# CristianSimion5/vk-raytracing-engine

Hardware: AMD Instinct MI355X
Metric: Mrays/s (higher is better)
Workload: dtype f32

## Files before the change

vk-raytracing-engine_amd/csrc/shade.h:

```cpp
#pragma once
#include "device_math.h"
#include "device_scene.h"
#include "texel.h"
#include "traverse.h"

struct Payload
{
  f3 hitValue;
  uint32_t seed;
  uint32_t depth;
  f3 rayOrigin, rayDirection, weight;
  bool isSpecular;
  float lightDist;
  f3 shadowRayDir;
};

struct ShadeStats
{
  unsigned hits, diffuse, taps;
  const float* lut;
};

VKRT_DEV const float* ldsTexelLut(const DevScene& sc, float* lds512)
{
  for(unsigned i = threadIdx.x; i < 512u; i += blockDim.x)
    lds512[i] = sc.srgbLut[i];
  __syncthreads();
  return lds512;
}

VKRT_DEV ShadeStats shadeStatsInit(const DevScene& sc, float* lds512)
{
  ShadeStats st;
  st.hits = 0; st.diffuse = 0; st.taps = 0;
  st.lut = ldsTexelLut(sc, lds512);
  return st;
}

VKRT_DEV f4 sampleTexLevel(const DevScene& sc, const DevTexture& tx, const uint32_t* levelOffsets, uint32_t level, float u, float v, const float* lut)
{
  const uint32_t ws = tx.width >> level, hs = tx.height >> level;
  const uint32_t w = ws ? ws : 1u, h = hs ? hs : 1u;
  TexTap tp;
  texFootprint(level == 0u ? tx.offset : levelOffsets[level], w, h, (tx.srgb & 1u) != 0u, true, true, u, v, tp);
  return texBlend(lut, tp, sc.texels[tp.i00], sc.texels[tp.i10], sc.texels[tp.i01], sc.texels[tp.i11]);
}

VKRT_DEV float lodLog2(float x)
{
  const uint32_t b = (uint32_t)__float_as_int(x);
  int e = (int)((b >> 23) & 255u) - 127;
  float m = __int_as_float((int)((b & 0x007fffffu) | 0x3f800000u));
  if(m > 1.41421356f)
  {
    m = m * 0.5f;
    e += 1;
  }
  const float s = (m - 1.0f) / (m + 1.0f), s2 = s * s;
  const float series = 1.0f + s2 * (0.333333333f + s2 * (0.2f + s2 * (0.142857143f + s2 * 0.111111111f)));
  return (float)e + (2.0f * s * series) * 1.44269504f;
}

struct TexGrad
{
  float dudx, dvdx, dudy, dvdy;
  bool on;
};

VKRT_DEV f4 sampleTex(const DevScene& sc, int texIndex, float u, float v, const TexGrad& g, ShadeStats& st)
{
  st.taps++;
  f4 r;
  if(sc.textureCount == 0u || texIndex < 0 || texIndex >= (int)sc.textureCount)
  {
    r.x = r.y = r.z = r.w = 1.0f;
    return r;
  }
  DevTexture tx = sc.textures[texIndex];
  const uint32_t levels = tx.srgb >> 8;
  if(!g.on || levels <= 1u)
    return sampleTexLevel(sc, tx, nullptr, 0u, u, v, st.lut);
  const uint32_t* levelOffsets = sc.texMips + (size_t)texIndex * VKRT_MAX_MIPS;
  const float fw = (float)tx.width, fh = (float)tx.height;
  const float mxu = g.dudx * fw, mxv = g.dvdx * fh, myu = g.dudy * fw, myv = g.dvdy * fh;
  const float rx2 = mxu * mxu + mxv * mxv, ry2 = myu * myu + myv * myv;
  const bool majorX = rx2 >= ry2;
  const float rmax = sqrtf(majorX ? rx2 : ry2), rmin = sqrtf(majorX ? ry2 : rx2);
  float eta = 1.0f;
  if(rmin > 0.0f)
    eta = glsl_min(rmax / rmin, 4.0f);
  else if(rmax > 0.0f)
    eta = 4.0f;
  if(!(eta >= 1.0f))
    eta = 1.0f;
  const int N = (int)ceilf(eta);
  const float scale = rmax / eta;
  float lambda = 0.0f;
  if(scale > 1.0f && scale < 3.0e38f)
    lambda = lodLog2(scale);
  else if(!(scale <= 1.0f))
    lambda = (float)(levels - 1u);
  lambda = glsl_clamp(lambda, 0.0f, (float)(levels - 1u));
  const float fl = floorf(lambda), delta = lambda - fl;
  const uint32_t hi = (uint32_t)fl, lo = hi + 1u < levels ? hi + 1u : levels - 1u;
  const float du = majorX ? g.dudx : g.dudy, dv = majorX ? g.dvdx : g.dvdy;
  r.x = r.y = r.z = r.w = 0.0f;
  for(int i = 1; i <= N; i++)
  {
    const float o = (float)i / (float)(N + 1) - 0.5f;
    float tu = u + o * du, tv = v + o * dv;
    if(!(fabsf(tu) < 1.0e9f) || !(fabsf(tv) < 1.0e9f))
    {
      tu = u;
      tv = v;
    }
    const f4 a = sampleTexLevel(sc, tx, levelOffsets, hi, tu, tv, st.lut), b = sampleTexLevel(sc, tx, levelOffsets, lo, tu, tv, st.lut);
    r.x = r.x + (a.x * (1.0f - delta) + b.x * delta);
    r.y = r.y + (a.y * (1.0f - delta) + b.y * delta);
    r.z = r.z + (a.z * (1.0f - delta) + b.z * delta);
    r.w = r.w + (a.w * (1.0f - delta) + b.w * delta);
  }
  const float inv = 1.0f / (float)N;
  r.x = r.x * inv; r.y = r.y * inv; r.z = r.z * inv; r.w = r.w * inv;
  return r;
}

VKRT_DEV f3 pbrGetBaseColor(const DevScene& sc, const GltfPBRMaterial& mat, float tu, float tv, const TexGrad& g, ShadeStats& st)
{
  f3 color = mk3(mat.pbrBaseColorFactor[0], mat.pbrBaseColorFactor[1], mat.pbrBaseColorFactor[2]);
  if(mat.pbrBaseColorTexture > -1)
  {
    const f4 t = sampleTex(sc, mat.pbrBaseColorTexture, tu, tv, g, st);
    color = color * mk3(t.x, t.y, t.z);
  }
  return color;
}
VKRT_DEV void pbrGetMetallicRoughness(const DevScene& sc, const GltfPBRMaterial& mat, float tu, float tv, const TexGrad& g,
                                      float& metallic, float& roughness, ShadeStats& st)
{
  metallic = mat.metallicFactor;
  roughness = mat.roughnessFactor;
  if(mat.metallicRoughnessTexture > -1)
  {
    const f4 t = sampleTex(sc, mat.metallicRoughnessTexture, tu, tv, g, st);
    roughness *= t.y;
    metallic *= t.z;
  }
}
VKRT_DEV float getNDF_GGXTR(f3 N, f3 H, float alpha)
{
  float a2 = alpha * alpha;
  float NH = dot3(N, H);
  if(NH <= 0.0f)
    return 0.0f;
  float NH2 = NH * NH;
  float d = NH2 * (a2 - 1.0f) + 1.0f;
  return a2 * VKRT_INV_PI / (d * d + 1e-4f);
}
VKRT_DEV float getG_SchlickGGX(float NV, float k) { return NV / (NV * (1.0f - k) + k); }
VKRT_DEV float getG_Smith(f3 N, f3 V, f3 L, float k)
{
  float NV = fabsf(dot3(N, V));
  float NL = fabsf(dot3(N, L));
  return getG_SchlickGGX(NV, k) * getG_SchlickGGX(NL, k);
}
VKRT_DEV f3 getF_Schlick(f3 H, f3 V, f3 F0)
{
  return F0 + (mk3(1.0f) - F0) * vk_pow5(1.0f - fabsf(dot3(H, V)));
}
VKRT_DEV f3 getSpecularBRDF_Cook_Torrance(f3 N, f3 H, f3 V, f3 L, f3 F0, float roughness)
{
  float alpha = roughness * roughness;
  float k = (roughness + 1.0f) * (roughness + 1.0f) / 8.0f;
  float D = getNDF_GGXTR(N, H, alpha);
  float G = getG_Smith(N, V, L, k);
  f3 F = getF_Schlick(H, V, F0);
  float down = 4.0f * fabsf(dot3(V, N)) * fabsf(dot3(L, N)) + 1e-4f;
  return D * F * G / down;
}
VKRT_DEV f3 getSpecularBRDF_over_pdf_Cook_Torrance(f3 N, f3 H, f3 V, f3 L, f3 F0, float roughness, float ratio)
{
  float k = (roughness + 1.0f) * (roughness + 1.0f) / 8.0f;
  float pdf = (1.0f - ratio) * dot3(N, H) / (4.0f * dot3(L, H) + 1e-4f);
  float G = getG_Smith(N, V, L, k);
  f3 F = getF_Schlick(H, V, F0);
  float down = 4.0f * fabsf(dot3(V, N)) * fabsf(dot3(L, N)) + 1e-4f;
  return (F * G / down) / pdf;
}
VKRT_DEV f3 computePBR_BRDF(f3 N, f3 V, f3 L, f3 H, f3 baseColor, float metalness, float roughness)
{
  f3 F0 = mk3(0.04f);
  F0 = glsl_mix(F0, baseColor, metalness);
  f3 F = getF_Schlick(H, V, F0);
  f3 f_cook_torrance = getSpecularBRDF_Cook_Torrance(N, H, V, L, F0, roughness);
  f3 kD = mk3(1.0f) - F;
  kD = kD * (1.0f - metalness);
  f3 f_lambert = baseColor * VKRT_INV_PI;
  f3 diffuse = kD * f_lambert;
  return diffuse + f_cook_torrance;
}
VKRT_DEV f3 directLight(const GltfLight& light, f3 P, f3 N, f3 V, f3 baseColor, float metalness, float roughness, unsigned retap,
                        f3& Li, float& cosTheta, ShadeStats& st)
{
  Li = mk3(0.0f);
  cosTheta = 0.0f;
  if(light.type == 0)
  {
    f3 Ldir = mk3(light.position[0], light.position[1], light.position[2]) - P;
    float d = length3(Ldir);
    f3 L = Ldir / d;
    f3 H = normalize3(L + V);
    float attenuation = d * d;
    Li = mk3(light.color[0], light.color[1], light.color[2]) * light.intensity / attenuation;
    cosTheta = glsl_max(dot3(L, N), 0.0f);
    if(cosTheta > 0.0f)
    {
      st.taps += retap;
      return computePBR_BRDF(N, V, L, H, baseColor, metalness, roughness);
    }
  }
  return mk3(0.0f);
}

VKRT_DEV f3 xformPoint(const DevInstance& in, f3 p)
{
  f3 r;
  r.x = ((in.o2w[0] * p.x + in.o2w[1] * p.y) + in.o2w[2] * p.z) + in.o2w[3];
  r.y = ((in.o2w[4] * p.x + in.o2w[5] * p.y) + in.o2w[6] * p.z) + in.o2w[7];
  r.z = ((in.o2w[8] * p.x + in.o2w[9] * p.y) + in.o2w[10] * p.z) + in.o2w[11];
  return r;
}
VKRT_DEV f3 xformNormal(const DevInstance& in, f3 n)
{
  f3 r;
  r.x = (n.x * in.w2o[0] + n.y * in.w2o[3]) + n.z * in.w2o[6];
  r.y = (n.x * in.w2o[1] + n.y * in.w2o[4]) + n.z * in.w2o[7];
  r.z = (n.x * in.w2o[2] + n.y * in.w2o[5]) + n.z * in.w2o[8];
  return r;
}

struct HitMid
{
  f3 worldPos, N, tangent, binormal, V, baseColor, emittance;
  float metalU, roughU;
  unsigned retap;
};

VKRT_DEV void closestHitFront(const DevScene& sc, const RayHit& hit, const uint32_t instId, const uint4 ts, f3 worldRayDir, const Payload& prd,
                              ShadeStats& st, HitMid& mid)
{
  st.hits++;
  const uint32_t i0 = ts.x, i1 = ts.y, i2 = ts.z, matIndex = ts.w;
  const f3 b = mk3(1.0f - hit.u - hit.v, hit.u, hit.v);

  const BufView vPN = bufView(sc.vertexPN), vMat = bufView(sc.shadeMaterials), vInst = bufView(sc.instances);
  const float4 a0 = bufLoad4(vPN, VKRT_VERTEX_BYTES * i0), b0 = bufLoad4(vPN, VKRT_VERTEX_BYTES * i0 + 16u), tq0 = bufLoad4(vPN, VKRT_VERTEX_BYTES * i0 + 32u);
  const float4 a1 = bufLoad4(vPN, VKRT_VERTEX_BYTES * i1), b1 = bufLoad4(vPN, VKRT_VERTEX_BYTES * i1 + 16u), tq1 = bufLoad4(vPN, VKRT_VERTEX_BYTES * i1 + 32u);
  const float4 a2 = bufLoad4(vPN, VKRT_VERTEX_BYTES * i2), b2 = bufLoad4(vPN, VKRT_VERTEX_BYTES * i2 + 16u), tq2 = bufLoad4(vPN, VKRT_VERTEX_BYTES * i2 + 32u);
  const uint32_t mo = 64u * matIndex;
  const float4 m0 = bufLoad4(vMat, mo), m1 = bufLoad4(vMat, mo + 16u), ref01 = bufLoad4(vMat, mo + 32u), ref23 = bufLoad4(vMat, mo + 48u);
  const uint32_t dimB = __float_as_uint(ref01.x), baseB = __float_as_uint(ref01.y), dimM = __float_as_uint(ref01.z), baseM = __float_as_uint(ref01.w);
  const uint32_t dimN = __float_as_uint(ref23.x), baseN = __float_as_uint(ref23.y), dimE = __float_as_uint(ref23.z), baseE = __float_as_uint(ref23.w);
  DevInstance in;
  {
    const uint32_t io = 96u * instId;
    const float4 q0 = bufLoad4(vInst, io), q1 = bufLoad4(vInst, io + 16u), q2 = bufLoad4(vInst, io + 32u), q3 = bufLoad4(vInst, io + 48u), q4 = bufLoad4(vInst, io + 64u),
                 q5 = bufLoad4(vInst, io + 80u);
    in.o2w[0] = q0.x; in.o2w[1] = q0.y; in.o2w[2] = q0.z; in.o2w[3] = q0.w; in.o2w[4] = q1.x; in.o2w[5] = q1.y; in.o2w[6] = q1.z; in.o2w[7] = q1.w;
    in.o2w[8] = q2.x; in.o2w[9] = q2.y; in.o2w[10] = q2.z; in.o2w[11] = q2.w;
    in.w2o[0] = q3.x; in.w2o[1] = q3.y; in.w2o[2] = q3.z; in.w2o[3] = q3.w; in.w2o[4] = q4.x; in.w2o[5] = q4.y; in.w2o[6] = q4.z; in.w2o[7] = q4.w;
    in.w2o[8] = q5.x; in.primMesh = __float_as_int(q5.y); in.vis = 0u; in.pad = 0;
  }
  GltfPBRMaterial mat;
  mat.pbrBaseColorFactor[0] = m0.x; mat.pbrBaseColorFactor[1] = m0.y; mat.pbrBaseColorFactor[2] = m0.z; mat.pbrBaseColorFactor[3] = 1.0f;
  mat.metallicFactor = m0.w; mat.roughnessFactor = m1.x;
  mat.emissiveFactor[0] = m1.y; mat.emissiveFactor[1] = m1.z; mat.emissiveFactor[2] = m1.w;
  mat.pbrBaseColorTexture = (dimB & 0x8000u) ? 0 : -1; mat.metallicRoughnessTexture = (dimM & 0x8000u) ? 0 : -1;
  mat.normalTexture = (dimN & 0x8000u) ? 0 : -1; mat.emissiveTexture = (dimE & 0x8000u) ? 0 : -1;
  const float tu = (b0.z * b.x + b1.z * b.y) + b2.z * b.z;
  const float tv = (b0.w * b.x + b1.w * b.y) + b2.w * b.z;

  const bool emits = prd.depth == 0 || prd.isSpecular;
  const bool wantE = emits && mat.emissiveTexture > -1, wantN = mat.normalTexture > -1;
  const bool wantB = mat.pbrBaseColorTexture > -1, wantM = mat.metallicRoughnessTexture > -1;
  st.taps += (wantE ? 1u : 0u) + (wantN ? 1u : 0u) + (wantB ? 1u : 0u) + (wantM ? 1u : 0u);
  TexTap tE, tN, tB, tM;
#define VKRT_FOOTPRINT(dim, base, want, tap)                                                                                           \
  texFootprint(sc.texQuads ? 0u : ((base) & 0x7fffffffu), ((dim) & 0x7fffu) + 1u, (((dim) >> 16) & 0x7fffu) + 1u, ((base) >> 31) != 0u, \
               ((dim) >> 31) != 0u, want, tu, tv, tap)
  VKRT_FOOTPRINT(dimE, baseE, wantE, tE);
  VKRT_FOOTPRINT(dimN, baseN, wantN, tN);
  VKRT_FOOTPRINT(dimB, baseB, wantB, tB);
  VKRT_FOOTPRINT(dimM, baseM, wantM, tM);
#undef VKRT_FOOTPRINT
  uint32_t e00, e10, e01, e11, n00, n10, n01, n11, c00, c10, c01, c11, r00, r10, r01, r11;
  if(sc.texQuads)
  {
    const BufView quads = bufView(sc.texQuads);
#define VKRT_QUAD(dim, base, tap, want, a, b, c, d)                                                                                    \
  {                                                                                                                                    \
    const uint32_t rec_ = ((want) && ((dim) >> 31) != 0u) ? tap.i00 + ((base) & 0x7fffffffu) : 0u;                                        \
    const float4 v_ = bufLoad4(quads, 16u * rec_);                                                                                     \
    a = __float_as_uint(v_.x); b = __float_as_uint(v_.y); c = __float_as_uint(v_.z); d = __float_as_uint(v_.w);                        \
  }
    VKRT_QUAD(dimE, baseE, tE, wantE, e00, e10, e01, e11)
    VKRT_QUAD(dimN, baseN, tN, wantN, n00, n10, n01, n11)
    VKRT_QUAD(dimB, baseB, tB, wantB, c00, c10, c01, c11)
    VKRT_QUAD(dimM, baseM, tM, wantM, r00, r10, r01, r11)
#undef VKRT_QUAD
  }
  else
  {
    const BufView tex = bufView(sc.texels);
#define VKRT_TEXEL(i) bufLoad1(tex, 4u * (i))
    e00 = VKRT_TEXEL(tE.i00); e10 = VKRT_TEXEL(tE.i10); e01 = VKRT_TEXEL(tE.i01); e11 = VKRT_TEXEL(tE.i11);
    n00 = VKRT_TEXEL(tN.i00); n10 = VKRT_TEXEL(tN.i10); n01 = VKRT_TEXEL(tN.i01); n11 = VKRT_TEXEL(tN.i11);
    c00 = VKRT_TEXEL(tB.i00); c10 = VKRT_TEXEL(tB.i10); c01 = VKRT_TEXEL(tB.i01); c11 = VKRT_TEXEL(tB.i11);
    r00 = VKRT_TEXEL(tM.i00); r10 = VKRT_TEXEL(tM.i10); r01 = VKRT_TEXEL(tM.i01); r11 = VKRT_TEXEL(tM.i11);
#undef VKRT_TEXEL
  }

  const f3 pos = mk3(a0.x, a0.y, a0.z) * b.x + mk3(a1.x, a1.y, a1.z) * b.y + mk3(a2.x, a2.y, a2.z) * b.z;
  const f3 worldPos = xformPoint(in, pos);
  const f3 nrm = normalize3(mk3(a0.w, b0.x, b0.y) * b.x + mk3(a1.w, b1.x, b1.y) * b.y + mk3(a2.w, b2.x, b2.y) * b.z);
  const f3 worldNrm = normalize3(xformNormal(in, nrm));
  const f3 tag = normalize3(mk3(tq0.x, tq0.y, tq0.z) * b.x + mk3(tq1.x, tq1.y, tq1.z) * b.y + mk3(tq2.x, tq2.y, tq2.z) * b.z);
  f3 worldTag = normalize3(xformNormal(in, tag));
  worldTag = normalize3(worldTag - dot3(worldTag, worldNrm) * worldNrm);
  const f3 worldBin = tq0.w * cross3(worldNrm, worldTag);

  f3 emittance = mk3(0.0f);
  if(emits)
  {
    emittance = mk3(mat.emissiveFactor[0], mat.emissiveFactor[1], mat.emissiveFactor[2]);
    if(wantE)
    {
      const f4 t = texBlend(st.lut, tE, e00, e10, e01, e11);
      emittance = emittance * mk3(t.x, t.y, t.z);
    }
  }
  f3 tangent = worldTag, binormal = worldBin;
  f3 texNormal = worldNrm;
  if(wantN)
  {
    const f4 t = texBlend(st.lut, tN, n00, n10, n01, n11);
    texNormal = normalize3(mk3(t.x, t.y, t.z) * 2.0f - mk3(1.0f));
    texNormal = normalize3(tangent * texNormal.x + binormal * texNormal.y + worldNrm * texNormal.z);
    createCoordinateSystem(texNormal, tangent, binormal);
  }
  f3 baseColor = mk3(mat.pbrBaseColorFactor[0], mat.pbrBaseColorFactor[1], mat.pbrBaseColorFactor[2]);
  if(wantB)
  {
    const f4 t = texBlend(st.lut, tB, c00, c10, c01, c11);
    baseColor = baseColor * mk3(t.x, t.y, t.z);
  }
  float metalness = mat.metallicFactor, roughness = mat.roughnessFactor;
  if(wantM)
  {
    const f4 t = texBlend(st.lut, tM, r00, r10, r01, r11);
    roughness *= t.y;
    metalness *= t.z;
  }

  mid.worldPos = worldPos; mid.N = texNormal; mid.tangent = tangent; mid.binormal = binormal;
  mid.V = normalize3(-worldRayDir);
  mid.baseColor = baseColor; mid.emittance = emittance;
  mid.metalU = metalness; mid.roughU = roughness;
  mid.retap = (mat.pbrBaseColorTexture > -1 ? 1u : 0u) + (mat.metallicRoughnessTexture > -1 ? 1u : 0u);
}

VKRT_DEV bool closestHitLobe(const HitMid& mid, Payload& prd)
{
  const float ratio = 0.5f * (1.0f - mid.metalU);
  const float r1 = rnd(prd.seed);
  return r1 < ratio;
}

VKRT_DEV void closestHitTail(const DevScene& sc, const PushConstantRay& pc, const HitMid& mid, const bool diffuse, Payload& prd, ShadeStats& st)
{
  const f3 worldPos = mid.worldPos, texNormal = mid.N, tangent = mid.tangent, binormal = mid.binormal, V = mid.V, N = mid.N;
  const f3 baseColor = mid.baseColor;
  f3 emittance = mid.emittance;
  const float metalU = mid.metalU, roughU = mid.roughU;
  const unsigned retap = mid.retap;
  const float ratio = 0.5f * (1.0f - metalU);
  const float roughness = glsl_clamp(roughU, 0.01f, 0.99f);
  const float metalness = glsl_clamp(metalU, 0.01f, 0.99f);
  const f3 rayOrigin = worldPos;
  f3 rayDirection;
  float pdf;
  f3 BRDF;
  if(diffuse)
  {
    st.diffuse++;
    prd.isSpecular = false;
    const int random_index = (int)(rnd(prd.seed) * (float)pc.lightsCount);
    const float4* lq = (const float4*)&sc.lights[random_index];
    const float4 l0 = lq[0], l1 = lq[1];
    GltfLight light;
    light.position[0] = l0.x; light.position[1] = l0.y; light.position[2] = l0.z;
    light.color[0] = l0.w; light.color[1] = l1.x; light.color[2] = l1.y;
    light.intensity = l1.z; light.type = __float_as_int(l1.w);
    const f3 lightDir = mk3(light.position[0], light.position[1], light.position[2]) - worldPos;
    const float lightDistance = length3(lightDir);
    const f3 L = normalize3(lightDir);
    prd.lightDist = lightDistance;
    prd.shadowRayDir = L;
    if(dot3(L, texNormal) <= 0)
      emittance = emittance + mk3(0.0f);
    else
    {
      f3 Li;
      float cosTheta;
      const f3 brdf = directLight(light, worldPos, texNormal, V, baseColor, metalU, roughU, retap, Li, cosTheta, st);
      emittance = emittance + (float)pc.lightsCount * brdf * Li * cosTheta;
    }
    rayDirection = normalize3(samplingHemisphere(prd.seed, tangent, binormal, texNormal));
    pdf = ratio * dot3(rayDirection, texNormal) * VKRT_INV_PI;
    BRDF = (1.0f - metalness) * baseColor * VKRT_INV_PI;
  }
  else
  {
    prd.isSpecular = true;
    const float alpha = roughness * roughness;
    const f3 h = samplingNDF_GGXTR(prd.seed, alpha * alpha);
    const f3 H = normalize3(tangent * h.x + binormal * h.y + texNormal * h.z);
    const f3 L = normalize3(glsl_reflect(-V, H));
    rayDirection = L;
    f3 F0 = mk3(0.04f);
    F0 = glsl_mix(F0, baseColor, metalness);
    pdf = 1.0f;
    BRDF = getSpecularBRDF_over_pdf_Cook_Torrance(N, H, V, L, F0, roughness, ratio);
  }
  const float cosTheta = dot3(rayDirection, texNormal);
  prd.rayOrigin = rayOrigin;
  prd.rayDirection = rayDirection;
  prd.hitValue = emittance;
  prd.weight = BRDF * cosTheta / pdf;
}

VKRT_DEV void closestHitShaderInst(const DevScene& sc, const PushConstantRay& pc, const RayHit& hit, const uint32_t instId, const uint4 ts,
                                   f3 worldRayDir, Payload& prd, ShadeStats& st)
{
  HitMid mid;
  closestHitFront(sc, hit, instId, ts, worldRayDir, prd, st, mid);
  const bool diffuse = closestHitLobe(mid, prd);
  closestHitTail(sc, pc, mid, diffuse, prd, st);
}

VKRT_DEV void closestHitShader(const DevScene& sc, const PushConstantRay& pc, const RayHit& hit, const uint4 ts, f3 worldRayDir, Payload& prd,
                               ShadeStats& st)
{
  const uint32_t instId = (uint32_t)__float_as_int(sc.tris[hit.slot * VKRT_TRI_QUADS + 2].z);
  closestHitShaderInst(sc, pc, hit, instId, ts, worldRayDir, prd, st);
}
VKRT_DEV void closestHitShader(const DevScene& sc, const PushConstantRay& pc, const RayHit& hit, f3 worldRayDir, Payload& prd, ShadeStats& st)
{
  closestHitShader(sc, pc, hit, sc.triShade[hit.slot], worldRayDir, prd, st);
}

VKRT_DEV void missShader(const PushConstantRay& pc, Payload& prd)
{
  if(prd.depth == 0)
    prd.hitValue = mk3(pc.clearColor[0], pc.clearColor[1], pc.clearColor[2]) * 0.8f;
  else
    prd.hitValue = mk3(0.01f);
  prd.depth = 100;
}

VKRT_DEV void mat4MulVec4(const float* M, float v0, float v1, float v2, float v3, float* out)
{
#pragma unroll
  for(int i = 0; i < 4; i++)
// ... 3 lines not shown
```

vk-raytracing-engine_amd/csrc/texel.h:

```cpp
#pragma once
#include "device_math.h"
#include "device_scene.h"

struct f4 { float x, y, z, w; };

typedef unsigned vkrt_v4u __attribute__((ext_vector_type(4)));
struct BufView { __amdgpu_buffer_rsrc_t r; };
VKRT_DEV BufView bufView(const void* p) { return BufView{__builtin_amdgcn_make_buffer_rsrc((void*)p, 0, (int)0xffffffffu, 0x00020000)}; }
VKRT_DEV float4 bufLoad4(BufView b, uint32_t byteOffset)
{
  const vkrt_v4u v = __builtin_amdgcn_raw_buffer_load_b128(b.r, (int)byteOffset, 0, 0);
  return make_float4(__uint_as_float(v.x), __uint_as_float(v.y), __uint_as_float(v.z), __uint_as_float(v.w));
}
VKRT_DEV uint32_t bufLoad1(BufView b, uint32_t byteOffset) { return __builtin_amdgcn_raw_buffer_load_b32(b.r, (int)byteOffset, 0, 0); }

VKRT_DEV int wrapi(int i, int n)
{
  if((n & (n - 1)) == 0)
    return i & (n - 1);
  int m = i % n;
  return m < 0 ? m + n : m;
}

struct TexTap
{
  uint32_t i00, i10, i01, i11;
  float ax, ay;
  uint32_t lutBase;
  bool white;
};
VKRT_DEV void texFootprint(uint32_t offset, uint32_t width, uint32_t height, bool srgb, bool valid, bool want, float u, float v, TexTap& t)
{
  float fx = u * (float)width - 0.5f;
  float fy = v * (float)height - 0.5f;
  if(!(fabsf(fx) < 1.0e9f)) fx = 0.0f;
  if(!(fabsf(fy) < 1.0e9f)) fy = 0.0f;
  const float flx = floorf(fx), fly = floorf(fy);
  t.ax = fx - flx; t.ay = fy - fly;
  const int w = (int)width, h = (int)height;
  const int x0 = wrapi((int)flx, w), y0 = wrapi((int)fly, h);
  const int x1 = x0 + 1 == w ? 0 : x0 + 1, y1 = y0 + 1 == h ? 0 : y0 + 1;
  const bool live = want && valid;
  const uint32_t r0 = offset + (uint32_t)y0 * width, r1 = offset + (uint32_t)y1 * width;
  t.i00 = live ? r0 + (uint32_t)x0 : 0u; t.i10 = live ? r0 + (uint32_t)x1 : 0u;
  t.i01 = live ? r1 + (uint32_t)x0 : 0u; t.i11 = live ? r1 + (uint32_t)x1 : 0u;
  t.lutBase = srgb ? 0u : 256u;
  t.white = !valid;
}
VKRT_DEV f4 texelDecode(const float* lut, uint32_t p, uint32_t base)
{
  f4 o;
  o.x = lut[base + (p & 255u)]; o.y = lut[base + ((p >> 8) & 255u)]; o.z = lut[base + ((p >> 16) & 255u)];
  o.w = lut[256u + (p >> 24)];
  return o;
}
VKRT_DEV f4 texBlend(const float* lut, const TexTap& tp, uint32_t p00, uint32_t p10, uint32_t p01, uint32_t p11)
{
  f4 r;
  if(tp.white)
  {
    r.x = r.y = r.z = r.w = 1.0f;
    return r;
  }
  const f4 t00 = texelDecode(lut, p00, tp.lutBase), t10 = texelDecode(lut, p10, tp.lutBase);
  const f4 t01 = texelDecode(lut, p01, tp.lutBase), t11 = texelDecode(lut, p11, tp.lutBase);
  const float ax = tp.ax, ay = tp.ay, bx = 1.0f - ax, by = 1.0f - ay;
  r.x = (t00.x * bx + t10.x * ax) * by + (t01.x * bx + t11.x * ax) * ay;
  r.y = (t00.y * bx + t10.y * ax) * by + (t01.y * bx + t11.y * ax) * ay;
  r.z = (t00.z * bx + t10.z * ax) * by + (t01.z * bx + t11.z * ax) * ay;
  r.w = (t00.w * bx + t10.w * ax) * by + (t01.w * bx + t11.w * ax) * ay;
  return r;
}

VKRT_DEV void texcoordAt(const float4 q0, const float4 q1, const float4 q2, const float u, const float v, float& tu, float& tv)
{
  const f3 b = mk3(1.0f - u - v, u, v);
  tu = (q0.z * b.x + q1.z * b.y) + q2.z * b.z;
  tv = (q0.w * b.x + q1.w * b.y) + q2.w * b.z;
}

template <bool PLAIN> struct TabView;
template <> struct TabView<false> { BufView b; };
template <> struct TabView<true> { const char* p; };
template <bool PLAIN>
VKRT_DEV TabView<PLAIN> tabView(const void* table)
{
  if constexpr(PLAIN)
    return TabView<true>{(const char*)table};
  else
    return TabView<false>{bufView(table)};
}
VKRT_DEV float4 tabLoad4(TabView<false> t, uint32_t byteOffset) { return bufLoad4(t.b, byteOffset); }
VKRT_DEV float4 tabLoad4(TabView<true> t, uint32_t byteOffset) { return *(const float4*)(t.p + byteOffset); }
VKRT_DEV uint32_t tabLoad1(TabView<false> t, uint32_t byteOffset) { return bufLoad1(t.b, byteOffset); }
VKRT_DEV uint32_t tabLoad1(TabView<true> t, uint32_t byteOffset) { return *(const uint32_t*)(t.p + byteOffset); }

template <bool LAZY>
VKRT_DEV float materialAlpha(const DevScene& sc, const uint32_t matIndex, const float tu, const float tv, const float* lut)
{
  const float factor = __uint_as_float(tabLoad1(tabView<LAZY>(sc.materials), 128u * matIndex + 12u));
  const float4 ref01 = tabLoad4(tabView<LAZY>(sc.shadeMaterials), 64u * matIndex + 32u);
  const uint32_t dimB = __float_as_uint(ref01.x), baseB = __float_as_uint(ref01.y);
  const bool wantB = (dimB & 0x8000u) != 0u;
  if(LAZY && !wantB)
    return factor;
  TexTap tB;
  texFootprint(sc.texQuads ? 0u : (baseB & 0x7fffffffu), (dimB & 0x7fffu) + 1u, ((dimB >> 16) & 0x7fffu) + 1u, (baseB >> 31) != 0u, (dimB >> 31) != 0u, wantB,
               tu, tv, tB);
  uint32_t c00, c10, c01, c11;
  if(sc.texQuads)
  {
    const uint32_t rec = (wantB && (dimB >> 31) != 0u) ? tB.i00 + (baseB & 0x7fffffffu) : 0u;
    const float4 q = tabLoad4(tabView<LAZY>(sc.texQuads), 16u * rec);
    c00 = __float_as_uint(q.x); c10 = __float_as_uint(q.y); c01 = __float_as_uint(q.z); c11 = __float_as_uint(q.w);
  }
  else
  {
    const TabView<LAZY> tex = tabView<LAZY>(sc.texels);
    c00 = tabLoad1(tex, 4u * tB.i00); c10 = tabLoad1(tex, 4u * tB.i10); c01 = tabLoad1(tex, 4u * tB.i01); c11 = tabLoad1(tex, 4u * tB.i11);
  }
  if(!wantB)
    return factor;
  return factor * texBlend(lut, tB, c00, c10, c01, c11).w;
}
```

vk-raytracing-engine_amd/csrc/wavefront.hip:

```cpp
#include <hip/hip_runtime.h>
#include <algorithm>
#include <cstdlib>
#include <cstring>

#include "device_math.h"
#include "device_scene.h"
#include "kernels.h"
#include "rgen.h"
#include "hybrid_gi.h"
#include "shade.h"
#include "traverse.h"
#include "traverse_wide.h"
#include "traverse_share.h"

#define WF_BLOCK 256
#define VKRT_FLAG_COUNT_WORK 2u

#include "wf_streams.h"

VKRT_DEV unsigned packFlags(const LaneState& L)
{
  return (L.prd.depth & 0xffu) | (((unsigned)L.smpl & 0xffffu) << 8) | ((L.prd.isSpecular ? 1u : 0u) << 25);
}

VKRT_DEV void loadCommon(const TraceParams& P, const WfBuffers& B, int parity, int type, unsigned i, LaneState& L)
{
  const float4 s0 = wfLoad(rec(B, parity, type, WF_S0, i)), s1 = wfLoad(rec(B, parity, type, WF_S1, i)), s2 = wfLoad(rec(B, parity, type, WF_S2, i));
  const unsigned flags = __float_as_uint(s1.w), pix = __float_as_uint(s2.w);
  L.curWeight = mk3(s0.x, s0.y, s0.z); L.prd.seed = __float_as_uint(s0.w);
  L.hitValue = mk3(s1.x, s1.y, s1.z);
  L.prd.depth = flags & 0xffu; L.smpl = (int)((flags >> 8) & 0xffffu);
  L.prd.isSpecular = ((flags >> 25) & 1u) != 0u;
  L.hitValues = mk3(s2.x, s2.y, s2.z);
  L.px = pix & 0xffffu; L.lrow = pix >> 16;
  L.camOrigin = cameraOrigin(P);
  L.prd.lightDist = 0.0f;
  L.prd.shadowRayDir = mk3(0.0f);
  L.prd.hitValue = mk3(0.0f);
  L.prd.weight = mk3(0.0f);
  L.stage = 0;
}

VKRT_DEV void storeState(const WfBuffers& B, int parity, int type, unsigned i, const LaneState& L, f3 weight)
{
  wfStore(rec(B, parity, type, WF_S0, i), make_float4(weight.x, weight.y, weight.z, __uint_as_float(L.prd.seed)));
  wfStore(rec(B, parity, type, WF_S1, i), make_float4(L.hitValue.x, L.hitValue.y, L.hitValue.z, __uint_as_float(packFlags(L))));
  wfStore(rec(B, parity, type, WF_S2, i), make_float4(L.hitValues.x, L.hitValues.y, L.hitValues.z, __uint_as_float(L.px | (L.lrow << 16))));
}

VKRT_DEV void storeClosest(const WfBuffers& B, int parity, unsigned i, const LaneState& L)
{
  wfStore(rec(B, parity, WF_C, WF_R0, i), make_float4(L.prd.rayOrigin.x, L.prd.rayOrigin.y, L.prd.rayOrigin.z, 10000.0f));
  wfStore(rec(B, parity, WF_C, WF_R1, i), make_float4(L.prd.rayDirection.x, L.prd.rayDirection.y, L.prd.rayDirection.z, 0.0f));
  storeState(B, parity, WF_C, i, L, L.curWeight);
}

VKRT_DEV void storeShadow(const WfBuffers& B, int parity, int type, unsigned i, const LaneState& L, f3 contrib, f3 nextWeight)
{
  wfStore(rec(B, parity, type, WF_R0, i), make_float4(L.prd.rayOrigin.x, L.prd.rayOrigin.y, L.prd.rayOrigin.z, L.prd.lightDist - 0.1f));
  wfStore(rec(B, parity, type, WF_R1, i), make_float4(L.prd.shadowRayDir.x, L.prd.shadowRayDir.y, L.prd.shadowRayDir.z, L.prd.lightDist));
  if(type == WF_P)
    wfStore(rec(B, parity, type, WF_R2, i), make_float4(L.prd.rayDirection.x, L.prd.rayDirection.y, L.prd.rayDirection.z, 0.0f));
  storeState(B, parity, type, i, L, nextWeight);
  wfStore(rec(B, parity, type, WF_S3, i), make_float4(contrib.x, contrib.y, contrib.z, 0.0f));
}

VKRT_DEV int finishSegment(const TraceParams& P, const WfBuffers& B, LaneState& L, bool shadowHit, f3 contrib, f3 nextWeight)
{
  const SegmentStep step = stepSegment(P, L, shadowHit, contrib, nextWeight);
  if(step == SEG_SAMPLE_END)
  {
    if(P.flags & VKRT_FLAG_SAMPLE_SYNC)
    {
      wfStore(B.sampleState + pixelSlot(P, L.px, L.lrow), make_float4(L.hitValues.x, L.hitValues.y, L.hitValues.z, __uint_as_float(L.prd.seed)));
      return -1;
    }
    startSample(P, L);
  }
  return step == SEG_PIXEL_DONE ? -1 : WF_C;
}

VKRT_DEV unsigned claimSlots(const WfBuffers& B, int parity, int to, unsigned lane, unsigned* wsum)
{
  const unsigned wave = threadIdx.x >> 6, nw = blockDim.x >> 6;
  const unsigned long long m[WF_TYPES] = {__ballot(to == WF_C), __ballot(to == WF_S), __ballot(to == WF_P)};
  if(lane == 0)
  {
#pragma unroll
    for(int t = 0; t < WF_TYPES; t++) wsum[t * (nw + 1) + wave] = (unsigned)__popcll(m[t]);
  }
  __syncthreads();
  if(threadIdx.x < WF_TYPES)
  {
    unsigned* w = wsum + threadIdx.x * (nw + 1);
    unsigned tot = 0;
    for(unsigned k = 0; k < nw; k++)
    {
      const unsigned c = w[k];
      w[k] = tot;
      tot += c;
    }
    w[nw] = tot ? atomicAdd(countOf(B, parity, (int)threadIdx.x), tot) : 0u;
  }
  __syncthreads();
  if(to < 0)
    return 0u;
  const unsigned long long below = (1ull << lane) - 1ull;
  const unsigned long long mine = to == WF_C ? m[0] : to == WF_S ? m[1] : m[2];
  return wsum[to * (nw + 1) + nw] + wsum[to * (nw + 1) + wave] + (unsigned)__popcll(mine & below);
}

__global__ __launch_bounds__(WF_BLOCK) void k_wf_init(const TraceParams P, const WfBuffers B)
{
  const unsigned lane = lane_id();
  const unsigned w = blockIdx.x * blockDim.x + threadIdx.x;
  bool alive = false;
  unsigned nPixels = 0;
  LaneState L;
  uint32_t x, y, lrow;
  if(pixelOfWork(P, w, P.tileFirst, x, y, lrow))
  {
    startPixel(P, L, x, y, lrow);
    nPixels = 1;
    if(P.pc.samples <= 0 || P.pc.depth <= 0)
      storePixel(P, L);
    else
      alive = true;
  }
  __shared__ unsigned wsum[WF_TYPES * (WF_BLOCK / 64 + 1)];
  const unsigned slot = claimSlots(B, 0, alive ? WF_C : -1, lane, wsum);
  if(alive)
    storeClosest(B, 0, slot, L);
  __shared__ unsigned long long red[VKRT_COUNTER_STRIDE * (WF_BLOCK / 64)];
  const unsigned vals[6] = {0, 0, 0, 0, 0, nPixels};
  blockAddCounters(&P.counters->v[blockIdx.x % VKRT_COUNTER_SLOTS][0], vals, 6, red);
}

__global__ __launch_bounds__(WF_BLOCK) void k_wf_sample_init(const TraceParams P, const WfBuffers B, const int round, const int smpl)
{
  const unsigned lane = lane_id();
  const unsigned w = blockIdx.x * blockDim.x + threadIdx.x;
  bool alive = false;
  LaneState L;
  uint32_t x, y, lrow;
  if(pixelOfWork(P, w, P.tileFirst, x, y, lrow))
  {
    const float4 st = wfLoad(B.sampleState + pixelSlot(P, x, lrow));
    bindPixel(P, L, x, lrow);
    L.prd.seed = __float_as_uint(st.w);
    L.hitValues = mk3(st.x, st.y, st.z);
    L.smpl = smpl;
    startSample(P, L);
    alive = true;
  }
  __shared__ unsigned wsum[WF_TYPES * (WF_BLOCK / 64 + 1)];
  const unsigned slot = claimSlots(B, round & 1, alive ? WF_C : -1, lane, wsum);
  if(alive)
    storeClosest(B, round & 1, slot, L);
}

VKRT_DEV bool advanceSegmentHybrid(const TraceParams& P, const HybridGi& G, LaneState& L, bool shadowHit, f3 contrib, f3 nextWeight, float lightDist)
{
  L.stage = 0;
  if(giSegmentStep(P.pc, L.prd, L.curWeight, L.hitValue, L.hitValues.x, shadowHit, contrib, nextWeight, lightDist))
    return true;
  hybridStorePixel(P, G, (size_t)L.lrow * P.fullW + L.px, true, L.hitValue, L.hitValues.x, L.hitValues.y);
  return false;
}

struct ShadeLds
{
  float lut[512];
  unsigned wsum[WF_TYPES * (WF_BLOCK / 64 + 1)];
};

template <bool PAIR, bool HYBRID, bool CAMERA = false>
VKRT_DEV void shadeHitBlock(const TraceParams& P, const WfBuffers& B, const HybridGi& G, const int par, const unsigned count, const unsigned block, ShadeLds& lds,
                            const int smpl = 0)
{
  const int type = PAIR ? WF_P : WF_C;
  const unsigned lane = lane_id();
  const unsigned qi = block * WF_BLOCK + threadIdx.x;
  ShadeStats st = shadeStatsInit(P.sc, lds.lut);
  unsigned* wsum = lds.wsum;
  int to = -1;
  LaneState L;
  f3 contrib = mk3(0.0f), nextWeight = mk3(0.0f);
  uint32_t x = 0, y = 0, lrow = 0;
  if(CAMERA ? pixelOfWork(P, qi, P.tileFirst, x, y, lrow) : qi < count)
  {
    if(CAMERA)
    {
      bindPixel(P, L, x, lrow);
      if(smpl == 0)
      {
        L.prd.seed = pixelSeed(P, x, y);
        L.hitValues = mk3(0.0f);
      }
      else
      {
        const float4 s = wfLoad(B.sampleState + pixelSlot(P, x, lrow));
        L.prd.seed = __float_as_uint(s.w);
        L.hitValues = mk3(s.x, s.y, s.z);
      }
      L.smpl = smpl;
      startSample(P, L);
    }
    else
      loadCommon(P, B, par, type, qi, L);
    const float4 h = wfLoad(rec(B, par, type, WF_H0, qi)), t4 = wfLoad(rec(B, par, type, WF_H1, qi));
    if(!CAMERA)
    {
      const float4 rd = wfLoad(rec(B, par, type, PAIR ? WF_R2 : WF_R1, qi));
      L.prd.rayDirection = mk3(rd.x, rd.y, rd.z);
    }
    L.prd.rayOrigin = mk3(0.0f);
    if(PAIR)
    {
      const float4 s3 = wfLoad(rec(B, par, WF_P, WF_S3, qi));
      const bool shadowHit = __float_as_int(h.x) != 0;
      if(HYBRID)
        (void)advanceSegmentHybrid(P, G, L, shadowHit, mk3(s3.x, s3.y, s3.z), L.curWeight, L.prd.depth == 1u ? wfLoad(rec(B, par, WF_P, WF_R1, qi)).w : 0.0f);
      else
        (void)advanceSegment(P, L, shadowHit, mk3(s3.x, s3.y, s3.z), L.curWeight);
    }
    RayHit hit;
    hit.t = h.x; hit.u = h.y; hit.v = h.z; hit.slot = __float_as_int(h.w);
    const uint4 ts = make_uint4(__float_as_uint(t4.x), __float_as_uint(t4.y), __float_as_uint(t4.z), __float_as_uint(t4.w));
    if(hit.slot >= 0)
      closestHitShaderInst(P.sc, P.pc, hit, (uint32_t)hit.slot, ts, L.prd.rayDirection, L.prd, st);
    else
      missShader(P.pc, L.prd);
    segmentTerms(L.prd, L.curWeight, contrib, nextWeight);
    const bool dead = !HYBRID && (P.flags & VKRT_FLAG_SKIP_DEAD_SHADOW) != 0u && contrib.x == 0.0f && contrib.y == 0.0f && contrib.z == 0.0f;
    if(!L.prd.isSpecular && L.prd.depth != 100u && !dead)
      to = (L.prd.depth + 1u < (uint32_t)P.pc.depth) ? WF_P : WF_S;
    else if(HYBRID)
      to = advanceSegmentHybrid(P, G, L, false, contrib, nextWeight, 0.0f) ? WF_C : -1;
    else
      to = finishSegment(P, B, L, false, contrib, nextWeight);
  }
  const unsigned slot = claimSlots(B, par ^ 1, to, lane, wsum);
  if(to == WF_C)
    storeClosest(B, par ^ 1, slot, L);
  else if(to >= 0)
    storeShadow(B, par ^ 1, to, slot, L, contrib, nextWeight);
  if(P.flags & VKRT_FLAG_COUNT_WORK)
  {
    __shared__ unsigned long long red[VKRT_COUNTER_STRIDE * (WF_BLOCK / 64)];
    const unsigned vals[5] = {0, 0, st.hits, st.diffuse, st.taps};
    blockAddCounters(&P.counters->v[blockIdx.x % VKRT_COUNTER_SLOTS][0], vals, 5, red);
  }
}

template <bool HYBRID>
VKRT_DEV void shadeShadowBlock(const TraceParams& P, const WfBuffers& B, const HybridGi& G, const int par, const unsigned count, const unsigned block, ShadeLds& lds)
{
  const unsigned lane = lane_id();
  const unsigned qi = block * WF_BLOCK + threadIdx.x;
  unsigned* wsum = lds.wsum;
  bool toClosest = false;
  LaneState L;
  if(qi < count)
  {
    loadCommon(P, B, par, WF_S, qi, L);
    const float4 h = wfLoad(rec(B, par, WF_S, WF_H0, qi)), s3 = wfLoad(rec(B, par, WF_S, WF_S3, qi));
    L.prd.rayOrigin = mk3(0.0f);
    L.prd.rayDirection = mk3(0.0f);
    const bool shadowHit = __float_as_int(h.w) >= 0;
    if(HYBRID)
      toClosest = advanceSegmentHybrid(P, G, L, shadowHit, mk3(s3.x, s3.y, s3.z), L.curWeight, L.prd.depth == 1u ? wfLoad(rec(B, par, WF_S, WF_R1, qi)).w : 0.0f);
    else
      toClosest = finishSegment(P, B, L, shadowHit, mk3(s3.x, s3.y, s3.z), L.curWeight) == WF_C;
  }
  const unsigned slot = claimSlots(B, par ^ 1, toClosest ? WF_C : -1, lane, wsum);
  if(toClosest)
    storeClosest(B, par ^ 1, slot, L);
}

template <bool HYBRID>
VKRT_DEV void shadeRound(const TraceParams& P, const WfBuffers& B, const HybridGi& G, const int round)
{
  const int par = round & 1;
  const unsigned cC = *countOf(B, par, WF_C), cS = *countOf(B, par, WF_S), cP = *countOf(B, par, WF_P);
  const unsigned nC = (cC + WF_BLOCK - 1) / WF_BLOCK, nP = (cP + WF_BLOCK - 1) / WF_BLOCK, nS = (cS + WF_BLOCK - 1) / WF_BLOCK;
  unsigned blk = blockIdx.x;
  __shared__ ShadeLds lds;
  if(blk < nC)
    shadeHitBlock<false, HYBRID>(P, B, G, par, cC, blk, lds);
  else if((blk -= nC) < nP)
    shadeHitBlock<true, HYBRID>(P, B, G, par, cP, blk, lds);
  else if((blk -= nP) < nS)
    shadeShadowBlock<HYBRID>(P, B, G, par, cS, blk, lds);
}
__global__ __launch_bounds__(WF_BLOCK) void k_wf_shade(const TraceParams P, const WfBuffers B, const int round)
{
  const HybridGi none{};
  shadeRound<false>(P, B, none, round);
}
__global__ __launch_bounds__(WF_BLOCK) void k_wf_shade_hybrid(const TraceParams P, const WfBuffers B, const HybridGi G, const int round)
{
  shadeRound<true>(P, B, G, round);
}
__global__ __launch_bounds__(WF_BLOCK) void k_wf_shade_camera(const TraceParams P, const WfBuffers B, const int round, const int smpl)
{
  const HybridGi none{};
  __shared__ ShadeLds lds;
  shadeHitBlock<false, false, true>(P, B, none, round & 1, 0u, blockIdx.x, lds, smpl);
}

__global__ __launch_bounds__(WF_BLOCK) void k_hy_gi_init(const TraceParams P, const WfBuffers B, const HybridGi G, const uint2* tmp)
{
  const unsigned lane = lane_id();
  const unsigned w = blockIdx.x * blockDim.x + threadIdx.x;
  bool alive = false;
  LaneState L;
  uint32_t x, y, lrow;
  if(pixelOfWork(P, w, P.tileFirst, x, y, lrow))
  {
    const size_t p = (size_t)lrow * P.fullW + x;
    const GbufferPixel g = loadGbufferPixel(G, p);
    const uint2 t = tmp[p];
    const float alpha = __uint_as_float(t.y);
    if(g.shaded)
    {
      bindPixel(P, L, x, lrow);
      L.prd.seed = t.x;
      giFirstRay(P, g, L.prd, L.curWeight);
      L.hitValue = mk3(0.0f);
      L.hitValues = mk3(0.0f, alpha, 0.0f);
      L.smpl = 0;
      L.stage = 0;
      alive = L.prd.depth < (uint32_t)P.pc.depth;
    }
    if(!alive)
      hybridStorePixel(P, G, p, g.shaded, mk3(0.0f), 0.0f, alpha);
  }
  __shared__ unsigned wsum[WF_TYPES * (WF_BLOCK / 64 + 1)];
  const unsigned slot = claimSlots(B, 0, alive ? WF_C : -1, lane, wsum);
  if(alive)
    storeClosest(B, 0, slot, L);
}

__global__ __launch_bounds__(WF_BLOCK) void k_wf_blend(const TraceParams P, const float4* stage)
{
  uint32_t x, y, lrow;
  if(pixelOfWork(P, blockIdx.x * blockDim.x + threadIdx.x, P.tileFirst, x, y, lrow))
  {
    const size_t p = (size_t)lrow * P.fullW + x;
    blendPixel((float4*)P.image + p, stage[p], P.pc.frame);
  }
}

#define WF_CTRL_BYTES (256 * VKRT_WF_MAX_LANES)
size_t vkrt_wf_state_bytes(uint32_t pathCapacity, int groups)
{
  const size_t g = (size_t)std::max(groups, 1);
  return g * pathCapacity * 2 * WF_SLOTS * sizeof(float4) + (g > 1 ? g * pathCapacity * sizeof(float4) : 0) + g * pathCapacity * sizeof(float4) +
         WF_CTRL_BYTES;
}

void vkrt_wf_carve(void* base, uint32_t pathCapacity, int groups, WfBuffers* B)
{
  const size_t g = (size_t)std::max(groups, 1);
  char* p = (char*)base;
  B->ctrl = (unsigned*)p;
  p += WF_CTRL_BYTES;
  B->planes = (float4*)p;
  p += g * pathCapacity * 2 * WF_SLOTS * sizeof(float4);
  B->stage = g > 1 ? (float4*)p : nullptr;
  p += g > 1 ? g * pathCapacity * sizeof(float4) : 0;
  B->sampleState = (float4*)p;
  B->capacity = pathCapacity;
  B->groups = (uint32_t)g;
}

static unsigned pixelBlocks(const TraceParams& P) { return (P.tileCount * 64u + WF_BLOCK - 1) / WF_BLOCK; }
static hipError_t subframeBegin(const TraceParams& P, const WfBuffers& B, bool init, hipStream_t stream)
{
  const hipError_t e = hipMemsetAsync(B.ctrl, 0, 64, stream);
  if(e == hipSuccess && init)
    hipLaunchKernelGGL(k_wf_init, dim3(pixelBlocks(P)), dim3(WF_BLOCK), 0, stream, P, B);
  return e;
}
static void launchTraverse(const TraceParams& P, const WfBuffers& B, int r, unsigned travBlock, bool count, hipStream_t stream)
{
  const unsigned work = P.tileCount * 64u, tb = (travBlock == 256u || travBlock == 128u) ? travBlock : 64u;
  vkrt_wf_launch_traverse(P, B, r, tb, count, dim3(2 * ((work + tb - 1) / tb) + 4), (size_t)P.sc.stackCap * tb * sizeof(int), stream);
}
static void subframeRound(const TraceParams& P, const WfBuffers& B, int r, int cameraSample, unsigned travBlock, bool count, hipStream_t stream, WfTiming* timing)
{
  const bool timed = timing && timing->events && 2 * (timing->used + 1) <= timing->capacity;
  if(timed)
    (void)hipEventRecord(timing->events[2 * timing->used], stream);
  if(cameraSample >= 0)
    vkrt_wf_launch_traverse_camera(P, B, r, cameraSample, count, (size_t)P.sc.stackCap * 64u * sizeof(int), stream);
  else
    launchTraverse(P, B, r, travBlock, count, stream);
  if(timed)
  {
    (void)hipEventRecord(timing->events[2 * timing->used + 1], stream);
    timing->used++;
  }
  if(cameraSample >= 0)
    hipLaunchKernelGGL(k_wf_shade_camera, dim3(pixelBlocks(P)), dim3(WF_BLOCK), 0, stream, P, B, r, cameraSample);
  else
    hipLaunchKernelGGL(k_wf_shade, dim3(pixelBlocks(P) + 3), dim3(WF_BLOCK), 0, stream, P, B, r);
}

hipError_t vkrt_launch_wavefront(const TraceParams& P, const WfBuffers& B, const WfOptions& opt, int frames, uint32_t seedStep, bool count,
                                 hipStream_t stream, WfTiming* timing, const WfAsync* async)
{
  const WfCall call{P.pc.samples, P.pc.depth, (P.flags & VKRT_FLAG_SAMPLE_SYNC) != 0u, (P.flags & VKRT_FLAG_CAMERA_ROUNDS) != 0u, P.tileCount, frames,
                    opt.inFlight, opt.subframes, (int)B.groups, async ? async->count : 0, timing != nullptr};
  const WfLanes lanes = wfLanes(call);
  const int L = lanes.F * lanes.S;
  const bool staged = lanes.F > 1;
  if(staged && wfPoolEvents(lanes.frames) > async->poolSize)
    return hipErrorInvalidValue;
  hipStream_t laneStream[VKRT_WF_MAX_LANES];
  WfBuffers Bq[VKRT_WF_MAX_LANES];
  laneStream[0] = stream;
  Bq[0] = B;
  const size_t groupQuads = (size_t)2 * WF_SLOTS * B.capacity;
  for(int q = 0; L > 1 && q < L; q++)
  {
    const int g = q / lanes.S, j = q % lanes.S;
    const uint32_t tile0 = lanes.tileFirst(j);
    Bq[q].ctrl = B.ctrl + 64 * q;
    Bq[q].planes = B.planes + (size_t)g * groupQuads + (size_t)2 * WF_SLOTS * ((size_t)tile0 * 64u);
    Bq[q].stage = staged ? B.stage + (size_t)g * B.capacity : nullptr;
    Bq[q].sampleState = B.sampleState + (size_t)g * B.capacity;
    Bq[q].capacity = (lanes.tileFirst(j + 1) - tile0) * 64u;
    Bq[q].groups = 1;
    laneStream[q] = async->streams[q];
  }
  int forked = 0;
  auto joinLanes = [&]() {
    hipError_t first = hipSuccess;
    for(int q = 0; q < forked; q++)
    {
      hipError_t x = hipEventRecord(async->join[q], laneStream[q]);
      if(x == hipSuccess) x = hipStreamWaitEvent(stream, async->join[q], 0);
      if(x != hipSuccess)
      {
        (void)hipStreamSynchronize(laneStream[q]);
        if(first == hipSuccess) first = x;
      }
    }
    return first;
  };
  hipError_t e = hipSuccess;
  if(L > 1 && (e = hipEventRecord(async->fork, stream)) != hipSuccess) return e;
  for(int q = 0; L > 1 && q < L; q++)
  {
    if((e = hipStreamWaitEvent(laneStream[q], async->fork, 0)) != hipSuccess)
    {
// ... 72 lines not shown
```

Measured before the change: 5423.

## Skip wave-idle texture taps, unroll LUT staging, and disable packed FP32 in shade kernels

Result: faster. 5514, median of 6 (+1.7%).

```diff
diff --git a/vk-raytracing-engine_amd/csrc/shade.h b/vk-raytracing-engine_amd/csrc/shade.h
--- a/vk-raytracing-engine_amd/csrc/shade.h
+++ b/vk-raytracing-engine_amd/csrc/shade.h
@@ -29,11 +29,26 @@
   return lds512;
 }
 
+template <unsigned BLOCK>
+VKRT_DEV const float* ldsTexelLutBlock(const DevScene& sc, float* lds512)
+{
+  static_assert(512u % BLOCK == 0u, "the table is 512 entries");
+#pragma unroll
+  for(unsigned k = 0; k < 512u / BLOCK; k++)
+    lds512[threadIdx.x + k * BLOCK] = sc.srgbLut[threadIdx.x + k * BLOCK];
+  __syncthreads();
+  return lds512;
+}
+
+template <unsigned BLOCK = 0u>
 VKRT_DEV ShadeStats shadeStatsInit(const DevScene& sc, float* lds512)
 {
   ShadeStats st;
   st.hits = 0; st.diffuse = 0; st.taps = 0;
-  st.lut = ldsTexelLut(sc, lds512);
+  if constexpr(BLOCK != 0u)
+    st.lut = ldsTexelLutBlock<BLOCK>(sc, lds512);
+  else
+    st.lut = ldsTexelLut(sc, lds512);
   return st;
 }
 
@@ -285,40 +300,35 @@
   const bool wantB = mat.pbrBaseColorTexture > -1, wantM = mat.metallicRoughnessTexture > -1;
   st.taps += (wantE ? 1u : 0u) + (wantN ? 1u : 0u) + (wantB ? 1u : 0u) + (wantM ? 1u : 0u);
   TexTap tE, tN, tB, tM;
-#define VKRT_FOOTPRINT(dim, base, want, tap)                                                                                           \
-  texFootprint(sc.texQuads ? 0u : ((base) & 0x7fffffffu), ((dim) & 0x7fffu) + 1u, (((dim) >> 16) & 0x7fffu) + 1u, ((base) >> 31) != 0u, \
-               ((dim) >> 31) != 0u, want, tu, tv, tap)
-  VKRT_FOOTPRINT(dimE, baseE, wantE, tE);
-  VKRT_FOOTPRINT(dimN, baseN, wantN, tN);
-  VKRT_FOOTPRINT(dimB, baseB, wantB, tB);
-  VKRT_FOOTPRINT(dimM, baseM, wantM, tM);
-#undef VKRT_FOOTPRINT
-  uint32_t e00, e10, e01, e11, n00, n10, n01, n11, c00, c10, c01, c11, r00, r10, r01, r11;
-  if(sc.texQuads)
-  {
-    const BufView quads = bufView(sc.texQuads);
-#define VKRT_QUAD(dim, base, tap, want, a, b, c, d)                                                                                    \
+  uint32_t e00 = 0u, e10 = 0u, e01 = 0u, e11 = 0u, n00 = 0u, n10 = 0u, n01 = 0u, n11 = 0u;
+  uint32_t c00 = 0u, c10 = 0u, c01 = 0u, c11 = 0u, r00 = 0u, r10 = 0u, r01 = 0u, r11 = 0u;
+  const bool pool = sc.texQuads != nullptr;
+  const BufView gather = bufView(pool ? (const void*)sc.texQuads : (const void*)sc.texels);
+#define VKRT_TAP(dim, base, want, tap, a, b, c, d)                                                                                     \
+  if(__ballot(want) != 0ull)                                                                                                           \
   {                                                                                                                                    \
-    const uint32_t rec_ = ((want) && ((dim) >> 31) != 0u) ? tap.i00 + ((base) & 0x7fffffffu) : 0u;                                        \
-    const float4 v_ = bufLoad4(quads, 16u * rec_);                                                                                     \
-    a = __float_as_uint(v_.x); b = __float_as_uint(v_.y); c = __float_as_uint(v_.z); d = __float_as_uint(v_.w);                        \
-  }
-    VKRT_QUAD(dimE, baseE, tE, wantE, e00, e10, e01, e11)
-    VKRT_QUAD(dimN, baseN, tN, wantN, n00, n10, n01, n11)
-    VKRT_QUAD(dimB, baseB, tB, wantB, c00, c10, c01, c11)
-    VKRT_QUAD(dimM, baseM, tM, wantM, r00, r10, r01, r11)
-#undef VKRT_QUAD
-  }
-  else
-  {
-    const BufView tex = bufView(sc.texels);
-#define VKRT_TEXEL(i) bufLoad1(tex, 4u * (i))
-    e00 = VKRT_TEXEL(tE.i00); e10 = VKRT_TEXEL(tE.i10); e01 = VKRT_TEXEL(tE.i01); e11 = VKRT_TEXEL(tE.i11);
-    n00 = VKRT_TEXEL(tN.i00); n10 = VKRT_TEXEL(tN.i10); n01 = VKRT_TEXEL(tN.i01); n11 = VKRT_TEXEL(tN.i11);
-    c00 = VKRT_TEXEL(tB.i00); c10 = VKRT_TEXEL(tB.i10); c01 = VKRT_TEXEL(tB.i01); c11 = VKRT_TEXEL(tB.i11);
-    r00 = VKRT_TEXEL(tM.i00); r10 = VKRT_TEXEL(tM.i10); r01 = VKRT_TEXEL(tM.i01); r11 = VKRT_TEXEL(tM.i11);
-#undef VKRT_TEXEL
-  }
+    const uint32_t w_ = ((dim) & 0x7fffu) + 1u, h_ = (((dim) >> 16) & 0x7fffu) + 1u;                                                   \
+    const bool live_ = (want) && ((dim) >> 31) != 0u;                                                                                  \
+    int x0_, y0_;                                                                                                                      \
+    texFootprintOrigin(w_, h_, ((base) >> 31) != 0u, ((dim) >> 31) != 0u, tu, tv, tap, x0_, y0_);                                      \
+    if(pool)                                                                                                                           \
+    {                                                                                                                                  \
+      const uint32_t rec_ = live_ ? ((uint32_t)y0_ * w_ + (uint32_t)x0_) + ((base) & 0x7fffffffu) : 0u;                                 \
+      const float4 v_ = bufLoad4(gather, 16u * rec_);                                                                                  \
+      a = __float_as_uint(v_.x); b = __float_as_uint(v_.y); c = __float_as_uint(v_.z); d = __float_as_uint(v_.w);                      \
+    }                                                                                                                                  \
+    else                                                                                                                               \
+    {                                                                                                                                  \
+      texFootprintTexels((base) & 0x7fffffffu, w_, h_, live_, x0_, y0_, tap);                                                          \
+      a = bufLoad1(gather, 4u * tap.i00); b = bufLoad1(gather, 4u * tap.i10);                                                          \
+      c = bufLoad1(gather, 4u * tap.i01); d = bufLoad1(gather, 4u * tap.i11);                                                          \
+    }                                                                                                                                  \
+  }
+  VKRT_TAP(dimE, baseE, wantE, tE, e00, e10, e01, e11)
+  VKRT_TAP(dimN, baseN, wantN, tN, n00, n10, n01, n11)
+  VKRT_TAP(dimB, baseB, wantB, tB, c00, c10, c01, c11)
+  VKRT_TAP(dimM, baseM, wantM, tM, r00, r10, r01, r11)
+#undef VKRT_TAP
 
   const f3 pos = mk3(a0.x, a0.y, a0.z) * b.x + mk3(a1.x, a1.y, a1.z) * b.y + mk3(a2.x, a2.y, a2.z) * b.z;
   const f3 worldPos = xformPoint(in, pos);
diff --git a/vk-raytracing-engine_amd/csrc/texel.h b/vk-raytracing-engine_amd/csrc/texel.h
--- a/vk-raytracing-engine_amd/csrc/texel.h
+++ b/vk-raytracing-engine_amd/csrc/texel.h
@@ -29,7 +29,7 @@
   uint32_t lutBase;
   bool white;
 };
-VKRT_DEV void texFootprint(uint32_t offset, uint32_t width, uint32_t height, bool srgb, bool valid, bool want, float u, float v, TexTap& t)
+VKRT_DEV void texFootprintOrigin(uint32_t width, uint32_t height, bool srgb, bool valid, float u, float v, TexTap& t, int& x0, int& y0)
 {
   float fx = u * (float)width - 0.5f;
   float fy = v * (float)height - 0.5f;
@@ -37,15 +37,23 @@
   if(!(fabsf(fy) < 1.0e9f)) fy = 0.0f;
   const float flx = floorf(fx), fly = floorf(fy);
   t.ax = fx - flx; t.ay = fy - fly;
+  x0 = wrapi((int)flx, (int)width); y0 = wrapi((int)fly, (int)height);
+  t.lutBase = srgb ? 0u : 256u;
+  t.white = !valid;
+}
+VKRT_DEV void texFootprintTexels(uint32_t offset, uint32_t width, uint32_t height, bool live, int x0, int y0, TexTap& t)
+{
   const int w = (int)width, h = (int)height;
-  const int x0 = wrapi((int)flx, w), y0 = wrapi((int)fly, h);
   const int x1 = x0 + 1 == w ? 0 : x0 + 1, y1 = y0 + 1 == h ? 0 : y0 + 1;
-  const bool live = want && valid;
   const uint32_t r0 = offset + (uint32_t)y0 * width, r1 = offset + (uint32_t)y1 * width;
   t.i00 = live ? r0 + (uint32_t)x0 : 0u; t.i10 = live ? r0 + (uint32_t)x1 : 0u;
   t.i01 = live ? r1 + (uint32_t)x0 : 0u; t.i11 = live ? r1 + (uint32_t)x1 : 0u;
-  t.lutBase = srgb ? 0u : 256u;
-  t.white = !valid;
+}
+VKRT_DEV void texFootprint(uint32_t offset, uint32_t width, uint32_t height, bool srgb, bool valid, bool want, float u, float v, TexTap& t)
+{
+  int x0, y0;
+  texFootprintOrigin(width, height, srgb, valid, u, v, t, x0, y0);
+  texFootprintTexels(offset, width, height, want && valid, x0, y0, t);
 }
 VKRT_DEV f4 texelDecode(const float* lut, uint32_t p, uint32_t base)
 {
diff --git a/vk-raytracing-engine_amd/csrc/wavefront.hip b/vk-raytracing-engine_amd/csrc/wavefront.hip
--- a/vk-raytracing-engine_amd/csrc/wavefront.hip
+++ b/vk-raytracing-engine_amd/csrc/wavefront.hip
@@ -174,6 +174,19 @@
   unsigned wsum[WF_TYPES * (WF_BLOCK / 64 + 1)];
 };
 
+VKRT_DEV bool pixelOfWave(const TraceParams& P, unsigned w, unsigned tileFirst, uint32_t& x, uint32_t& y, uint32_t& lrow)
+{
+  if(w >= P.tileCount * 64u)
+    return false;
+  const unsigned tile = (unsigned)__builtin_amdgcn_readfirstlane((int)(tileFirst + (w >> 6))), inTile = w & 63u;
+  x = (tile % P.tilesX) * 8u + (inTile & 7u);
+  lrow = (tile / P.tilesX) * 8u + (inTile >> 3);
+  if(x >= P.fullW || lrow >= P.localRows)
+    return false;
+  y = globalRow(P, lrow);
+  return y < P.fullH;
+}
+
 template <bool PAIR, bool HYBRID, bool CAMERA = false>
 VKRT_DEV void shadeHitBlock(const TraceParams& P, const WfBuffers& B, const HybridGi& G, const int par, const unsigned count, const unsigned block, ShadeLds& lds,
                             const int smpl = 0)
@@ -181,13 +194,13 @@
   const int type = PAIR ? WF_P : WF_C;
   const unsigned lane = lane_id();
   const unsigned qi = block * WF_BLOCK + threadIdx.x;
-  ShadeStats st = shadeStatsInit(P.sc, lds.lut);
+  ShadeStats st = shadeStatsInit<WF_BLOCK>(P.sc, lds.lut);
   unsigned* wsum = lds.wsum;
   int to = -1;
   LaneState L;
   f3 contrib = mk3(0.0f), nextWeight = mk3(0.0f);
   uint32_t x = 0, y = 0, lrow = 0;
-  if(CAMERA ? pixelOfWork(P, qi, P.tileFirst, x, y, lrow) : qi < count)
+  if(CAMERA ? pixelOfWave(P, qi, P.tileFirst, x, y, lrow) : qi < count)
   {
     if(CAMERA)
     {
@@ -199,7 +212,7 @@
       }
       else
       {
-        const float4 s = wfLoad(B.sampleState + pixelSlot(P, x, lrow));
+        const float4 s = wfLoad(B.sampleState + (P.tileFirst * 64u + qi));
         L.prd.seed = __float_as_uint(s.w);
         L.hitValues = mk3(s.x, s.y, s.z);
       }
@@ -243,8 +256,10 @@
   const unsigned slot = claimSlots(B, par ^ 1, to, lane, wsum);
   if(to == WF_C)
     storeClosest(B, par ^ 1, slot, L);
-  else if(to >= 0)
-    storeShadow(B, par ^ 1, to, slot, L, contrib, nextWeight);
+  else if(to == WF_P)
+    storeShadow(B, par ^ 1, WF_P, slot, L, contrib, nextWeight);
+  else if(to == WF_S)
+    storeShadow(B, par ^ 1, WF_S, slot, L, contrib, nextWeight);
   if(P.flags & VKRT_FLAG_COUNT_WORK)
   {
     __shared__ unsigned long long red[VKRT_COUNTER_STRIDE * (WF_BLOCK / 64)];
@@ -278,6 +293,11 @@
     storeClosest(B, par ^ 1, slot, L);
 }
 
+#if defined(__HIP_DEVICE_COMPILE__)
+#define WF_SCALAR_FP32 __attribute__((target("no-packed-fp32-ops")))
+#else
+#define WF_SCALAR_FP32
+#endif
 template <bool HYBRID>
 VKRT_DEV void shadeRound(const TraceParams& P, const WfBuffers& B, const HybridGi& G, const int round)
 {
@@ -293,16 +313,16 @@
   else if((blk -= nP) < nS)
     shadeShadowBlock<HYBRID>(P, B, G, par, cS, blk, lds);
 }
-__global__ __launch_bounds__(WF_BLOCK) void k_wf_shade(const TraceParams P, const WfBuffers B, const int round)
+WF_SCALAR_FP32 __global__ __launch_bounds__(WF_BLOCK) void k_wf_shade(const TraceParams P, const WfBuffers B, const int round)
 {
   const HybridGi none{};
   shadeRound<false>(P, B, none, round);
 }
-__global__ __launch_bounds__(WF_BLOCK) void k_wf_shade_hybrid(const TraceParams P, const WfBuffers B, const HybridGi G, const int round)
+WF_SCALAR_FP32 __global__ __launch_bounds__(WF_BLOCK) void k_wf_shade_hybrid(const TraceParams P, const WfBuffers B, const HybridGi G, const int round)
 {
   shadeRound<true>(P, B, G, round);
 }
-__global__ __launch_bounds__(WF_BLOCK) void k_wf_shade_camera(const TraceParams P, const WfBuffers B, const int round, const int smpl)
+WF_SCALAR_FP32 __global__ __launch_bounds__(WF_BLOCK) void k_wf_shade_camera(const TraceParams P, const WfBuffers B, const int round, const int smpl)
 {
   const HybridGi none{};
   __shared__ ShadeLds lds;
```
